# jsansao/voice_synth

Hardware: AMD Instinct MI355X
Metric: synthesised Msamples/s (whole node) at 1/2/4/8 MI355X; RMS vs C ref (higher is better)
Workload: dtype f64

## Files before the change

### voice_synth_amd/csrc/vs_api.c

```c
#include <math.h>
#include <pthread.h>
#include <stdio.h>
#include <stdlib.h>
#include <string.h>
#include <time.h>
#include <unistd.h>

#include "vs_internal.h"

double vs_now_ms(void)
{
  struct timespec ts;
  clock_gettime(CLOCK_MONOTONIC, &ts);
  return 1e3 * (double)ts.tv_sec + 1e-6 * (double)ts.tv_nsec;
}

int vs_ctx_create(int device, vs_ctx **out)
{
  if (!out) return VS_ERR_ARG;
  *out = NULL;
  int count = 0;
  if (hipGetDeviceCount(&count) != hipSuccess || count <= 0) return VS_ERR_NODEVICE;
  if (device < 0 || device >= count) return VS_ERR_NODEVICE;
  hipDeviceProp_t prop;
// ... 366 lines not shown
    b->retired = NULL;
  }
}

int vs_plan_create_impl(vs_ctx *ctx, const vs_lane *lanes, size_t n_lanes, size_t n_samples,
                        int mode, vs_plan **out)
{
  const int filter_only = (mode & VS_PLAN_FILTER_ONLY) ? 1 : 0;
  const int zero_copy = (mode & VS_PLAN_ZERO_COPY) ? 1 : 0;
  if (!ctx || !lanes || !out || n_lanes == 0 || n_samples == 0) return VS_ERR_ARG;
  if (n_lanes > (size_t)0x7FFFFFC0 || n_samples > (size_t)0x7FFFFF00) return VS_ERR_UNSUPPORTED;
  *out = NULL;
  if (!zero_copy) {
    const int wrc = vs_copy_path_warm(ctx);
    if (wrc != VS_OK) return wrc;
  }
  const vs_tuning *tune = &ctx->tuning;
  int rc = VS_OK;
  if (!ctx->planws) {
    ctx->planws = vs_planws_create();
    vs_planws_set_big_allocator(ctx->planws, plan_pinned_alloc, plan_pinned_free, ctx);
  }
  if (!ctx->planws) return VS_ERR_NOMEM;
  VsDevLane *dl = NULL;
  double *costab = NULL;
  size_t costab_len = 0, costab_cap = 0;
  int *row_of_T2 = NULL;
  double *awide = NULL;
  void *small_tmp = NULL;
  VsGroupSlot *gmap = NULL;
  vs_plan *p = NULL;
  const double t_host0 = vs_now_ms();
  VsBatchStats st;
  rc = vs_expand_all_ordered_ws(ctx->planws, lanes, n_lanes, filter_only, &dl, NULL, &st);
  if (rc != VS_OK) goto done;

  int tmax = st.tmax;
  int min_lframe = st.min_lframe;
  const bool any_onoise = st.any_onoise != 0;
  if (!filter_only) {
    row_of_T2 = (int *)malloc(((size_t)st.max_T2 + 1) * sizeof(int));
    if (!row_of_T2) {
      rc = VS_ERR_NOMEM;
      goto done;
    }
    for (int t = 0; t <= st.max_T2; t++) row_of_T2[t] = -1;
    for (size_t l = 0; l < n_lanes; l++) {
      const int T2 = dl[l].T2;
      if (row_of_T2[T2] < 0) {
        if (costab_len + (size_t)T2 > costab_cap) {
          size_t cap = costab_cap ? 2 * costab_cap : 1024;
          while (cap < costab_len + (size_t)T2) cap *= 2;
          double *grown = (double *)realloc(costab, cap * sizeof(double));
          if (!grown) {
            rc = VS_ERR_NOMEM;
            goto done;
          }
          costab = grown;
          costab_cap = cap;
        }
        vs_cos_row(T2, &costab[costab_len]);
        row_of_T2[T2] = (int)costab_len;
        costab_len += (size_t)T2;
      }
      dl[l].tab_off = row_of_T2[T2];
    }
  }
// ... 554 lines not shown
```

### voice_synth_amd/csrc/vs_dev_filter.h

```cpp
#ifndef VS_DEV_FILTER_H
#define VS_DEV_FILTER_H

template <int ARITH>
__device__ __forceinline__ void vs_load_taps(const double *__restrict__ taps, const VsDevLane *__restrict__ L,
                                             double (&a)[VS_ORDER + 1])
{
  const double *__restrict__ row = taps + (size_t)L->tap_row * VS_ORDER;
  a[0] = 1.0;
#pragma unroll
  for (int j = 1; j <= VS_ORDER; ++j) {
    a[j] = (ARITH == VS_ARITH_FMA) ? -row[j - 1] : row[j - 1];
    if (ARITH == VS_ARITH_FMA) asm volatile("" : "+v"(a[j]));
  }
}

__device__ __forceinline__ void vs_unpack8(const vs_u32x4 v, int *x)
{
#pragma unroll
  for (int e = 0; e < 4; ++e) {
    x[2 * e] = (int)(int16_t)(v[e] & 0xFFFFu);
    x[2 * e + 1] = (int)v[e] >> 16;
  }
}

#define VS_ONDW_UNKNOWN 0x7FC00000u
struct VsFramePower {
  float sum;
  float done;
  int tb;
  int len;
  int frame;
  bool bad;
  bool requirk;
  bool force;
  const VsDevLane *lanes;
  float *ondw;
  long ondw_pitch;
  long first_lane;
  int n_lanes;
};
__device__ __forceinline__ double vs_sqrt_rn(double v)
{
  double s = sqrt(v);
  if (!(v > 0.0) || !(s > 0.0)) return s;
  const double r = __builtin_fma(-s, s, v);
  const double up = __longlong_as_double(__double_as_longlong(s) + 1) - s;
  const double dn = s - __longlong_as_double(__double_as_longlong(s) - 1);
  if (r > s * up) s = s + up;
  else if (-r > s * dn) s = s - dn;
  return s;
}
__device__ __forceinline__ float vs_noise_width(float aux, int ni, float snr)
{
  const float sig_power = aux / (float)ni;
  return (float)vs_sqrt_rn((double)(12.0f * sig_power / snr));
}
__device__ __forceinline__ void vs_power_pair(uint32_t w, float &aux)
{
  const float lo = (float)(int)(int16_t)(w & 0xFFFFu), hi = (float)((int)w >> 16);
  aux += lo * lo;
  aux += hi * hi;
}
__device__ __forceinline__ void vs_frame_power_store(const VsFramePower &fp, bool unknown)
{
  const long gl = fp.first_lane + (long)(threadIdx.x & (VS_WAVE - 1));
  if (gl < (long)fp.n_lanes) {
    const VsDevLane *__restrict__ L = fp.lanes + gl;
    const float snr = L->out_snr;
    if (snr > 0.0f)
      fp.ondw[(long)L->row * fp.ondw_pitch + fp.frame] = unknown ? __uint_as_float(VS_ONDW_UNKNOWN) : vs_noise_width(fp.done, fp.len, snr);
  }
}
__device__ __forceinline__ void vs_frame_power_mark(VsFramePower &fp, int t)
{
  const bool ends = fp.tb == t + 1;
  fp.done = ends ? fp.sum : fp.done;
  fp.sum = ends ? 0.0f : fp.sum;
}

template <int ARITH, int KIND, bool PRE1 = false, bool PACKED = false, int WHOLE = -1, bool LATE = false, bool POW = false>
__device__ __forceinline__ void vs_superstep(const double (&a)[VS_ORDER + 1], double (&y)[VS_SS],
                                             double gain, double pre, const int16_t *rp,
                                             const int16_t *__restrict__ irow,
                                             int16_t *__restrict__ orow, int n, int N, bool vec_ok,
                                             int (&outv)[VS_SS], vs_u32x4 (&xnext)[VS_SS / 8],
                                             bool store_ok = true, VsFramePower *fp = nullptr)
{
  static_assert(!POW || (PACKED && WHOLE == 1), "frame powers ride on the eager packing of the branch-free super-step");
  const bool whole = (WHOLE < 0) ? (vec_ok && (n + VS_SS <= N)) : (WHOLE != 0);
  int xin[VS_SS];
  if (KIND == VS_KIND_FILTER) {
    if (whole) {
#pragma unroll
      for (int k = 0; k < VS_SS / 8; ++k) vs_unpack8(xnext[k], &xin[8 * k]);
      if (n + 2 * VS_SS <= N) {
#pragma unroll
        for (int k = 0; k < VS_SS / 8; ++k) xnext[k] = *(const vs_u32x4 *)(irow + n + VS_SS + 8 * k);
      }
    } else {
#pragma unroll
      for (int t = 0; t < VS_SS; ++t) xin[t] = (n + t < N) ? (int)irow[n + t] : 0;
    }
  } else {
#pragma unroll
    for (int t = 0; t < 8; ++t) xin[t] = (int)rp[t * VS_GROUP_LANES];
  }

  constexpr bool EAGER = PACKED && (WHOLE == 1);
  constexpr int PKN = (EAGER && LATE) ? 12 : 4;
  uint32_t pk[PKN];
  auto put8 = [&](int k) {
    if (EAGER && LATE) {
      if (k == VS_SS / 8 - 1) {
#pragma unroll
        for (int c = 0; c < VS_SS / 8; ++c) {
          vs_u32x4 v;
#pragma unroll
          for (int e = 0; e < 4; ++e) v[e] = pk[(4 * c + e) % PKN];
          if (store_ok) *(vs_u32x4 *)(orow + n + 8 * c) = v;
        }
      }
    } else if (EAGER) {
      vs_u32x4 v;
#pragma unroll
      for (int e = 0; e < 4; ++e) v[e] = pk[e];
      if (store_ok) *(vs_u32x4 *)(orow + n + 8 * k) = v;
    } else if (whole) {
      vs_u32x4 v;
#pragma unroll
      for (int e = 0; e < 4; ++e)
        v[e] = PACKED ? vs_clamp_pack16(outv[8 * k + 2 * e], outv[8 * k + 2 * e + 1])
                      : vs_pack16(outv[8 * k + 2 * e], outv[8 * k + 2 * e + 1]);
      if (store_ok) *(vs_u32x4 *)(orow + n + 8 * k) = v;
    } else {
#pragma unroll
      for (int t = 8 * k; t < 8 * k + 8; ++t) {
        int v = outv[t];
        if (PACKED) v = (v > 32767) ? 32767 : ((v < -32767) ? -32767 : v);
        if (store_ok && (n + t < N)) orow[n + t] = (int16_t)v;
      }
    }
  };

  if (KIND == VS_KIND_SOURCE) {
#pragma unroll
    for (int t = 8; t < VS_SS; ++t) xin[t] = (int)rp[t * VS_GROUP_LANES];
#pragma unroll
    for (int t = 0; t < VS_SS; ++t) outv[t] = xin[t];
#pragma unroll
    for (int k = 0; k < VS_SS / 8; ++k) put8(k);
  } else {
    const double ym1 = y[VS_SS - 1];
    int qhi = 0x7FFFFFFF;
    uint32_t qlo = 0u;
#pragma unroll
    for (int t = 0; t < VS_SS; ++t) {
      if (KIND != VS_KIND_FILTER && (t & 7) == 0) {
        if (t + 8 < VS_SS) {
#pragma unroll
          for (int u = t + 8; u < t + 16; ++u) xin[u] = (int)rp[u * VS_GROUP_LANES];
        }
        asm volatile(".p2align 3" ::"v"(xin[t]), "v"(xin[t + 1]), "v"(xin[t + 2]), "v"(xin[t + 3]), "v"(xin[t + 4]),
                     "v"(xin[t + 5]), "v"(xin[t + 6]), "v"(xin[t + 7]));
      }
      double acc;
      const double y1 = y[(t + VS_SS - 1) % VS_SS];
      if (ARITH == VS_ARITH_EXACT) {
        acc = __builtin_fma((double)xin[t], gain, -(a[1] * y1));
#pragma unroll
        for (int j = 2; j <= VS_ORDER; ++j) acc = acc - a[j] * y[(t + VS_SS - j) % VS_SS];
      } else {
        acc = (double)xin[t] * gain;
        double p0 = acc, p1 = a[2] * y[(t + VS_SS - 2) % VS_SS];
#pragma unroll
        for (int j = 3; j <= VS_ORDER; ++j) {
          const double yj = y[(t + VS_SS - j) % VS_SS];
          if (j & 1) p0 = __builtin_fma(a[j], yj, p0);
          else p1 = __builtin_fma(a[j], yj, p1);
        }
        acc = __builtin_fma(a[1], y1, p0 + p1);
      }
      const double o = PRE1 ? (acc - y1)
                            : ((ARITH == VS_ARITH_EXACT) ? (acc - pre * y1) : __builtin_fma(-pre, y1, acc));
      if (ARITH == VS_ARITH_FMA && PACKED) {
        outv[t] = (int)__builtin_rint(o);
        asm volatile("" : "+v"(outv[t]));
      } else {
        outv[t] = PACKED ? vs_round2int_half_down_unclamped(o) : vs_round2int_half_down(o);
        asm volatile("" : "+v"(outv[t]));
        const int ohi = __double2hiint(o);
        const uint32_t olo = (uint32_t)__double2loint(o);
        qhi = (ohi < qhi) ? ohi : qhi;
        qlo = (olo > qlo) ? olo : qlo;
// ... 117 lines not shown
```

### voice_synth_amd/csrc/vs_kernels.hip

```cpp
#include <hip/hip_runtime.h>
#include <stdint.h>

#include "../../include/voice_synth.h"
#include "vs_device.h"

#include "vs_dev_primitives.h"
#include "vs_dev_generator.h"
#include "vs_dev_filter.h"


__device__ __forceinline__ void vs_load_cfg(const VsDevLane *__restrict__ L, VsCfg &c, VsGen &s)
{
  c.jitter = L->jitter; c.shimmer = L->shimmer; c.K = L->K; c.Kvar = L->Kvar;
  c.DC = L->DC; c.noise = L->noise; c.t_hi = L->t_hi; c.t_lo = L->t_lo;
  c.a_hi = L->a_hi; c.a_lo = L->a_lo;
  c.amp = L->amp; c.P = L->P; c.T2 = L->T2; c.tab_off = 0;
  c.dcs = L->dcs;
  c.thr = L->thr;
  c.flags = L->flags; c.key0 = L->key0; c.key1 = L->key1;
  s.d = 0u;
  s.dp0 = 0.0f; s.ds0 = 0.0f;
  s.T4 = 0; s.T = c.P; s.g = 0; s.wpos = 0; s.cyc = 0;
  s.amp_next = 0.0f; s.S_next = 0.0f; s.K_next = 0.0f; s.pend = false; s.posted = 0;
}
// ... 109 lines not shown
    VS_DIAG_ADD(dg, 6)
  }
#ifdef VS_DIAG
  if (args.diag && lane == 0) {
#pragma unroll
    for (int k = 0; k < 8; ++k) args.diag[(size_t)blockIdx.x * 8 + k] = dg.acc[k];
  }
#endif

  if (KIND != VS_KIND_FILTER && args.ncyc && valid) args.ncyc[row] = s.cyc;
}

#if VS_GROUP_LANES == VS_WAVE
#ifdef VS_POLL_SLEEP
#define VS_POLL_SLEEP_2 VS_POLL_SLEEP
#define VS_POLL_SLEEP_3 VS_POLL_SLEEP
#else
#define VS_POLL_SLEEP_2 32
#define VS_POLL_SLEEP_3 8
#endif
template <bool THREE>
__device__ __forceinline__ void vs_poll_sleep()
{
  if (THREE) __builtin_amdgcn_s_sleep(VS_POLL_SLEEP_3);
  else __builtin_amdgcn_s_sleep(VS_POLL_SLEEP_2);
}

struct VsGroup {
  const VsDevLane *L;
  int16_t *ring;
  double *ltab;
  int *gpub, *npub;
  VsOrderBox ord;
  long group, row;
  int lane, N, C;
  int ltab_entries;
  bool valid;
};

template <bool SPLIT>
__device__ __forceinline__ void vs_generator_wave(const VsKernelArgs &args, const VsGroup &g)
{
  const int lane = g.lane, N = g.N, C = g.C;
  VsCfg c;
  VsGen s;
  VsDiag dg;
#ifdef VS_DIAG
#pragma unroll
  for (int k = 0; k < 8; ++k) dg.acc[k] = 0;
  dg.rounds = dg.attend = 0;
  dg.t = vs_stamp();
#endif
  vs_load_cfg(g.L, c, s);
  vs_stage_cos_rows(g.L, c, g.ltab, args.costab, g.ltab_entries, lane, g.valid, args);
  __builtin_amdgcn_fence(__ATOMIC_RELEASE, "workgroup");
  VsRoundKeys rk;
  if (!SPLIT) vs_round_keys(c.key0, c.key1, rk);
  int spins = 0;
  int prev_seen = -1, prev_taken = -1;
  bool dirty = true;
  const bool withhold = args.fault == VS_FAULT_WITHHOLD_PROGRESS;
  while (!withhold) {
#ifdef VS_TIMING_GENERATOR_ONLY
    const int n_seen = s.g;
#else
    const int n_seen = __hip_atomic_load(&g.npub[lane], __ATOMIC_RELAXED, __HIP_MEMORY_SCOPE_WORKGROUP);
#endif
// ... 85 lines not shown
        taken += 1;
        VS_LDS_RELEASE();
        __hip_atomic_store(&g.ord.otak[lane], taken, __ATOMIC_RELAXED, __HIP_MEMORY_SCOPE_WORKGROUP);
        const int T3 = w1 & 0xFFFF, T = (int)((unsigned)w1 >> 16);
        const int m = T - T3;
        __hip_atomic_store(&g.gpub[lane], gend + T3, __ATOMIC_RELAXED, __HIP_MEMORY_SCOPE_WORKGROUP);
        if (__any(m > 0)) {
          vs_noise_trips<true, true>(g.ring, C, lane, rk, vs_noise_consts(NDW, dcs), d0, m, wpos, T3, gend,
                                     &g.gpub[lane]);
        }
        gend += T;
        wpos += T;
        if (wpos >= C) wpos -= C;
      }
      spins = 0;
      VS_DIAG_ADD(dg, 4)
    } else {
      vs_poll_sleep<true>();
      VS_DIAG_ADD(dg, 6)
      if (++spins > args.spin_limit) {
        if (args.err && lane == 0) atomicOr(args.err, 4);
        break;
      }
    }
  }
#ifdef VS_DIAG
  if (args.diag && lane == 0) {
    args.diag[(size_t)g.group * 16 + 11] = dg.acc[4];
    args.diag[(size_t)g.group * 16 + 12] = dg.acc[6];
  }
#endif
}

template <int ARITH, bool PRE1, bool PARTIAL, bool POW>
__device__ __forceinline__ void vs_filter_wave(const VsKernelArgs &args, const VsGroup &g)
{
  const int lane = g.lane, N = g.N, C = g.C;
  const VsDevLane *__restrict__ L = g.L;
  int16_t *ring = g.ring;
  int *gpub = g.gpub, *npub = g.npub;
  const bool valid = g.valid;
  if (args.ws_filter_prio >= 3) __builtin_amdgcn_s_setprio(3);
  else if (args.ws_filter_prio == 2) __builtin_amdgcn_s_setprio(2);
  else if (args.ws_filter_prio == 1) __builtin_amdgcn_s_setprio(1);
  constexpr bool F32 = (ARITH == VS_ARITH_F32);
  constexpr int DARITH = F32 ? VS_ARITH_FMA : ARITH;
  VsF32Filter f32;
  double a[VS_ORDER + 1];
  if (F32) vs_f32_load(args.taps, L, f32);
  else vs_load_taps<DARITH>(args.taps, L, a);
  const double gain = L->gain;
  const double pre = L->pre;
  int16_t *orow = args.out + g.row * args.out_pitch;
  const int ready_min = (args.ready_min > 0) ? args.ready_min : __builtin_amdgcn_readfirstlane(L->ready_min);
#ifdef VS_DIAG
  VsDiag dg;
#pragma unroll
  for (int k = 0; k < 8; ++k) dg.acc[k] = 0;
  dg.t = vs_stamp();
#endif
  if (!PARTIAL || ready_min >= VS_WAVE) {
    double y[VS_SS];
#pragma unroll
    for (int j = 0; j < VS_SS; ++j) y[j] = 0.0;
    bool gave_up = false;
    int rslot = 0;
    auto await = [&](int n) {
      for (int polls = 0; !gave_up; ++polls) {
#ifdef VS_TIMING_FILTER_ONLY
        const int g_seen = N;
#else
        const int g_seen = __hip_atomic_load(&gpub[lane], __ATOMIC_RELAXED, __HIP_MEMORY_SCOPE_WORKGROUP);
#endif
        const bool ready = !valid || (g_seen - n >= VS_SS) || (g_seen >= N);
        if (__all(ready)) break;
        vs_poll_sleep<!PARTIAL>();
        VS_DIAG_ADD(dg, 6)
        if (polls > args.spin_limit) {
          if (args.err && lane == 0) atomicOr(args.err, 2);
          gave_up = true;
        }
      }
      __builtin_amdgcn_fence(__ATOMIC_ACQUIRE, "workgroup");
    };
    auto release = [&](int n_done) {
      rslot += VS_SS;
      if (rslot >= C) rslot = 0;
      VS_LDS_RELEASE();
      __hip_atomic_store(&npub[lane], n_done, __ATOMIC_RELAXED, __HIP_MEMORY_SCOPE_WORKGROUP);
    };
    if (!valid) orow = args.sink;
    const int n_whole = (args.vec_ok != 0) ? (N / VS_SS) * VS_SS : 0;
    VsFramePower fp;
    int f_len = 0, f_left = 0;
    if (POW) {
      fp.sum = fp.done = 0.0f;
      fp.frame = 0;
      fp.bad = fp.requirk = false;
      fp.lanes = args.lanes;
      fp.ondw = args.ondw;
      fp.ondw_pitch = args.ondw_pitch;
      fp.first_lane = g.group * VS_WAVE;
      fp.n_lanes = args.n_lanes;
      f_len = f_left = (args.pow_lframe < N) ? args.pow_lframe : N;
    }
    int n = 0;
    for (; n < n_whole; n += VS_SS) {
      VS_DIAG_ADD(dg, 7)
      await(n);
      int outv[VS_SS];
      vs_u32x4 xpre[VS_SS / 8];
      if (POW) {
        fp.tb = (f_left <= VS_SS) ? f_left : 0;
        fp.len = f_len;
        fp.force = (args.fault == VS_FAULT_REROUND) && ((n / VS_SS) % 7 == 3);
      }
      if constexpr (F32)
        vs_superstep_f32<PRE1, 1, POW>(f32, ring + rslot * VS_WAVE + lane, orow, n, N, true, &fp);
      else
        vs_superstep<DARITH, VS_KIND_SYNTH, PRE1, true, 1, PARTIAL, POW>(a, y, gain, pre, ring + rslot * VS_WAVE + lane, nullptr, orow, n,
                                                                         N, true, outv, xpre, true, &fp);
      if (POW) {
        if (fp.tb) {
          vs_frame_power_store(fp, fp.bad || fp.requirk);
          fp.frame += 1;
          fp.bad = fp.requirk;
          const int rest = N - (n + fp.tb);
          f_len = (args.pow_lframe < rest) ? args.pow_lframe : rest;
          f_left = f_len - (VS_SS - fp.tb);
        } else {
          fp.bad = fp.bad || fp.requirk;
          f_left -= VS_SS;
        }
        fp.requirk = false;
      }
      release(n + VS_SS);
      VS_DIAG_ADD(dg, 0)
    }
    if (POW && valid) args.odone[g.row] = fp.frame;
    for (; n < N; n += VS_SS) {
      VS_DIAG_ADD(dg, 7)
      await(n);
      int outv[VS_SS];
      vs_u32x4 xpre[VS_SS / 8];
      if constexpr (F32)
        vs_superstep_f32<PRE1, 0, false>(f32, ring + rslot * VS_WAVE + lane, orow, n, N, true);
      else
        vs_superstep<DARITH, VS_KIND_SYNTH, PRE1, true, 0>(a, y, gain, pre, ring + rslot * VS_WAVE + lane, nullptr, orow, n,
                                                           N, false, outv, xpre, true);
      release(n + VS_SS);
      VS_DIAG_ADD(dg, 0)
    }
  } else {
    if (POW && valid) args.odone[g.row] = 0;
    double y[VS_SS];
#pragma unroll
    for (int j = 0; j < VS_SS; ++j) y[j] = 0.0;
    int n = 0, rslot = 0, spins = 0;
    bool live = valid;
    while (__any(live)) {
      VS_DIAG_ADD(dg, 7)
#ifdef VS_TIMING_FILTER_ONLY
      const int g_seen = N;
#else
      const int g_seen = __hip_atomic_load(&gpub[lane], __ATOMIC_RELAXED, __HIP_MEMORY_SCOPE_WORKGROUP);
#endif
      __builtin_amdgcn_fence(__ATOMIC_ACQUIRE, "workgroup");
      const bool ready = live && ((g_seen - n >= VS_SS) || (g_seen >= N));
      const int n_live = __builtin_popcountll(__ballot(live));
      const int n_ready = __builtin_popcountll(__ballot(ready));
      if ((n_ready > 0) && (n_ready * 64 >= n_live * ready_min)) {
        const bool inside = (args.vec_ok != 0) && (n + VS_SS <= N);
        if (__all(!ready || inside)) {
          if (ready) {
            int outv[VS_SS];
            vs_u32x4 xpre[VS_SS / 8];
            if constexpr (F32)
              vs_superstep_f32<PRE1, 1, false>(f32, ring + rslot * VS_WAVE + lane, orow, n, N, true);
            else
              vs_superstep<DARITH, VS_KIND_SYNTH, PRE1, true, 1, PARTIAL>(a, y, gain, pre, ring + rslot * VS_WAVE + lane, nullptr, orow,
                                                                          n, N, true, outv, xpre);
          }
        } else {
          if (ready) {
            int outv[VS_SS];
            vs_u32x4 xpre[VS_SS / 8];
            if constexpr (F32)
              vs_superstep_f32<PRE1, 0, false>(f32, ring + rslot * VS_WAVE + lane, orow, n, N, true);
            else
              vs_superstep<DARITH, VS_KIND_SYNTH, PRE1, true>(a, y, gain, pre, ring + rslot * VS_WAVE + lane, nullptr, orow,
                                                              n, N, args.vec_ok != 0, outv, xpre);
          }
        }
        if (ready) {
          rslot += VS_SS;
          if (rslot >= C) rslot = 0;
          n += VS_SS;
          if (n >= N) live = false;
        }
        VS_LDS_RELEASE();
        __hip_atomic_store(&npub[lane], n, __ATOMIC_RELAXED, __HIP_MEMORY_SCOPE_WORKGROUP);
        spins = 0;
        VS_DIAG_ADD(dg, 0)
      } else {
        vs_poll_sleep<!PARTIAL>();
        VS_DIAG_ADD(dg, 6)
        if (++spins > args.spin_limit) {
          if (args.err && lane == 0) atomicOr(args.err, 2);
          break;
        }
      }
    }
  }
#ifdef VS_DIAG
  if (args.diag && lane == 0) {
    args.diag[(size_t)g.group * 16 + 8] = dg.acc[0];
    args.diag[(size_t)g.group * 16 + 14] = dg.acc[6];
    args.diag[(size_t)g.group * 16 + 15] = dg.acc[7];
  }
#endif
}

template <int ARITH, bool PRE1, int ROLES, bool POW>
__device__ __forceinline__ void vs_synth_ws_body(const VsKernelArgs &args)
{
  extern __shared__ __attribute__((aligned(16))) int16_t lds_base[];

  const int widx = (int)threadIdx.x >> 6;
  int ngroups, role, slot;
  if (ROLES == 3 && args.ws_layout == VS_WS_LAYOUT_SPREAD_2X3) {
    const int simd = widx & 3, second = widx >> 2;
    ngroups = 2;
    slot = simd >> 1;
    role = (simd & 1) ? (second ? 1 : 0) : (second ? -1 : 2);
  } else {
    ngroups = (int)blockDim.x / (ROLES * VS_WAVE);
    role = widx / ngroups;
    slot = widx - role * ngroups;
  }
  VsGroup g;
  g.lane = (int)threadIdx.x & (VS_WAVE - 1);
  g.group = (long)blockIdx.x * (long)ngroups + slot;
  g.C = args.ring_slots;
  g.ltab_entries = args.ltab_entries;
  g.ring = lds_base + (size_t)slot * (size_t)(args.ws_pair_bytes / sizeof(int16_t));
  if (args.group_map) {
    const VsGroupSlot gs = args.group_map[(size_t)blockIdx.x * (size_t)ngroups + (size_t)slot];
    g.group = (gs.group >= 0) ? (long)gs.group : (((long)args.n_lanes + VS_WAVE - 1) / VS_WAVE);
    g.C = __builtin_amdgcn_readfirstlane(gs.ring_slots);
    g.ring = lds_base + (size_t)__builtin_amdgcn_readfirstlane(gs.lds_off) / sizeof(int16_t);
    g.ltab_entries = __builtin_amdgcn_readfirstlane(gs.ltab_entries);
  }
  const long gl = g.group * VS_WAVE + g.lane;
  g.valid = gl < (long)args.n_lanes;
  g.L = args.lanes + (g.valid ? gl : (long)args.n_lanes - 1);
  g.N = args.n_samples;
  g.ltab = (double *)(g.ring + (size_t)(g.C + VS_TRASH_ROWS) * VS_WAVE);
  g.gpub = (int *)(g.ltab + g.ltab_entries);
  g.npub = g.gpub + VS_WAVE;
  g.ord.oseq = g.npub + VS_WAVE;
  g.ord.otak = g.ord.oseq + VS_WAVE;
  g.ord.w = g.ord.otak + VS_WAVE;
  g.row = (long)g.L->row;

  if (role == 0) {
    g.gpub[g.lane] = 0;
    g.npub[g.lane] = 0;
    if (ROLES == 3) {
      g.ord.oseq[g.lane] = 0;
      g.ord.otak[g.lane] = 0;
    }
  }
  __syncthreads();
  if (role < 0) return;
  if (g.group * VS_WAVE >= (long)args.n_lanes) return;

#ifdef VS_TIMING_GENERATOR_ONLY
  if (role == ROLES - 1) return;
#endif
#ifdef VS_TIMING_FILTER_ONLY
  if (role != ROLES - 1) return;
#endif
  if (role == ROLES - 1) vs_filter_wave<ARITH, PRE1, ROLES == 2, POW>(args, g);
  else if (ROLES == 3 && role == 1) vs_noise_wave(args, g);
  else vs_generator_wave<ROLES == 3>(args, g);
}
template <int ARITH, bool PRE1, int ROLES>
__global__ void __launch_bounds__(ROLES * 4 * VS_WAVE) vs_synth_ws_kernel(VsKernelArgs args)
{
  vs_synth_ws_body<ARITH, PRE1, ROLES, false>(args);
}
template <int ARITH, bool PRE1, int ROLES>
__global__ void __launch_bounds__(ROLES * 4 * VS_WAVE) vs_synth_ws_pow_kernel(VsKernelArgs args)
{
  vs_synth_ws_body<ARITH, PRE1, ROLES, true>(args);
}

__device__ __forceinline__ void vs_power8(const vs_u32x4 v, float &aux)
{
#pragma unroll
  for (int e = 0; e < 4; ++e) {
    const float lo = (float)(int)(int16_t)(v[e] & 0xFFFFu), hi = (float)((int)v[e] >> 16);
    aux += lo * lo;
    aux += hi * hi;
  }
}

template <bool VEC>
__device__ __forceinline__ float vs_frame_width(const VsKernelArgs &args, const VsDevLane *__restrict__ L, long row, int fr, float snr)
{
  const int N = args.n_samples;
  const int Lframe = L->Lframe;
  const long f0 = (long)fr * Lframe;
  if (f0 >= N) return __uint_as_float(VS_ONDW_UNKNOWN);
  const int left = N - (int)f0;
  const int ni = (left < Lframe) ? left : Lframe;
// ... 565 lines not shown
```

### voice_synth_amd/csrc/vs_planhost.c

```c
#include <math.h>
#include <pthread.h>
#include <signal.h>
#include <stdlib.h>
#include <string.h>
#include <unistd.h>

#include "vs_planhost.h"

uint32_t vs_lframe_magic(int Lframe)
{
  if (Lframe < 2) return 0u;
  int k = 0;
  while (((uint64_t)1 << k) < (uint64_t)Lframe) k++;
  return (uint32_t)((((uint64_t)1 << (31 + k)) / (uint64_t)Lframe) + 1u);
}

int vs_lane_taps(const vs_lane *lane, double *A)
{
  for (int j = 0; j < VS_MAX_NCOEF; j++) A[j] = 0.0;
  if (lane->vowel != VS_VOWEL_CUSTOM) return vs_vowel_coefficients(lane->vowel, A);
  int order = 0;
  const int rc = vs_lane_order(lane, &order);
  if (rc != VS_OK) return rc;
  for (int j = 0; j <= order; j++) A[j] = lane->A[j];
// ... 114 lines not shown
  } else if (vs_vowel_index(lane->vowel) < 0) {
    return (lane->vowel == 'A' || lane->vowel == 'I' || lane->vowel == 'U') ? VS_ERR_UNSUPPORTED : VS_ERR_RANGE;
  }
  if (lane->fs <= 0) return VS_ERR_RANGE;
  memset(d, 0, sizeof(*d));
  d->tap_row = (lane->vowel == VS_VOWEL_CUSTOM) ? -1 : vs_vowel_index(lane->vowel);
  d->gain = (double)lane->gain;
  d->pre = (double)lane->pre_emphasis;
  d->row = row;
  d->out_snr = lane->out_snr;
  {
    const unsigned long nSamplesPerSec = (unsigned long)lane->fs;
    const int milisec1 = (int)(nSamplesPerSec * 0.001 / 2.0) * 2;
    d->Lframe = 50 * milisec1;
    d->lframe_magic = vs_lframe_magic(d->Lframe);
  }
  if (lane->out_snr > 0 && d->Lframe <= 0) return VS_ERR_UNSUPPORTED;
  d->okey0 = (uint32_t)lane->out_seed;
  d->okey1 = (uint32_t)(lane->out_seed >> 32);
  return VS_OK;
}

#define VS_EXPAND_THREADS 16
typedef struct ExpandJob {
  const vs_lane *lanes;
  VsDevLane *dl;
  const uint32_t *order;
  size_t lo, hi;
  int filter_only;
  int rc;
  size_t bad;
  VsBatchStats st;
  uint64_t *key;
  uint64_t key_or, key_and;
} ExpandJob;

static void stats_init(VsBatchStats *st)
{
  memset(st, 0, sizeof(*st));
  st->tmax = 1;
  st->pre1 = 1;
}
static void stats_lane(VsBatchStats *st, const vs_lane *lane, const VsDevLane *d)
{
  if (d->T2 > st->max_T2) st->max_T2 = d->T2;
  if (d->tbound > st->tmax) st->tmax = d->tbound;
  if (d->Lframe > 0 && (st->min_lframe == 0 || d->Lframe < st->min_lframe)) st->min_lframe = d->Lframe;
  if (d->Lframe > st->max_lframe) st->max_lframe = d->Lframe;
  if (d->Lframe <= 0) st->no_lframe = 1;
  if (d->out_snr > 0) st->any_onoise = 1;
  if (d->pre != 1.0) st->pre1 = 0;
  if (vs_lane_is_wide(lane)) st->wide = 1;
  if (d->tap_row < 0) st->n_custom++;
  if (d->flags & VS_DF_NOISE) st->n_noisy++;
}
static void stats_merge(VsBatchStats *a, const VsBatchStats *b)
{
  if (b->max_T2 > a->max_T2) a->max_T2 = b->max_T2;
  if (b->tmax > a->tmax) a->tmax = b->tmax;
  if (b->min_lframe > 0 && (a->min_lframe == 0 || b->min_lframe < a->min_lframe)) a->min_lframe = b->min_lframe;
  if (b->max_lframe > a->max_lframe) a->max_lframe = b->max_lframe;
  a->no_lframe |= b->no_lframe;
  a->any_onoise |= b->any_onoise;
  a->pre1 &= b->pre1;
  a->wide |= b->wide;
  a->n_noisy += b->n_noisy;
// ... 200 lines not shown
    rec_release(ws);
    ws->rec_big = (ws->big_alloc != NULL) && n >= VS_TEAM_MIN_LANES;
    ws->rec[0] = rec_alloc(ws, 0, n);
    if (!ws->rec[0]) return VS_ERR_NOMEM;
    ws->rec_lanes = n;
  }
  if (need_order) {
    if (!ws->rec[1]) {
      ws->rec[1] = rec_alloc(ws, 1, ws->rec_lanes);
      if (!ws->rec[1]) return VS_ERR_NOMEM;
    }
    if (ws->idx_lanes < n) {
      free(ws->idx[0]);
      free(ws->idx[1]);
      ws->idx_lanes = 0;
      ws->idx[0] = (uint32_t *)malloc(n * sizeof(uint32_t));
      ws->idx[1] = (uint32_t *)malloc(n * sizeof(uint32_t));
      if (!ws->idx[0] || !ws->idx[1]) return VS_ERR_NOMEM;
      ws->idx_lanes = n;
    }
    if (!ws->count) ws->count = (size_t *)malloc(65537 * sizeof(size_t));
    if (!ws->count) return VS_ERR_NOMEM;
  }
  if (ws->key_lanes < n) {
    free(ws->key);
    ws->key_lanes = 0;
    ws->key = (uint64_t *)malloc(n * sizeof(uint64_t));
    if (!ws->key) return VS_ERR_NOMEM;
    ws->key_lanes = n;
  }
  return VS_OK;
}

static uint64_t record_order_key(const VsDevLane *d)
{
  return ((uint64_t)(uint32_t)d->P << 36) | ((uint64_t)(uint32_t)d->T2 << 8) |
         (uint64_t)(d->flags & (VS_DF_JITTER | VS_DF_SHIMMER | VS_DF_NOISE));
}

static void expand_range(void *arg)
{
  ExpandJob *j = (ExpandJob *)arg;
  j->rc = VS_OK;
  j->bad = (size_t)-1;
  j->key_or = 0;
  j->key_and = ~(uint64_t)0;
  stats_init(&j->st);
  for (size_t i = j->lo; i < j->hi; i++) {
    const size_t l = j->order ? (size_t)j->order[i] : i;
    const int rc = j->filter_only ? vs_expand_filter_lane(&j->lanes[l], (int32_t)l, &j->dl[i])
                                  : vs_expand_lane(&j->lanes[l], (int32_t)l, &j->dl[i]);
    if (rc != VS_OK) {
      if (l < j->bad) {
        j->rc = rc;
        j->bad = l;
      }
      if (!j->order) break;
      continue;
    }
    stats_lane(&j->st, &j->lanes[l], &j->dl[i]);
    if (j->key) {
      const uint64_t k = record_order_key(&j->dl[i]);
      j->key[i] = k;
      j->key_or |= k;
      j->key_and &= k;
    }
  }
}

typedef struct GatherJob {
  const VsDevLane *in;
  VsDevLane *out;
  const uint32_t *order;
  size_t lo, hi;
} GatherJob;
static void gather_range(void *arg)
{
  GatherJob *j = (GatherJob *)arg;
  for (size_t i = j->lo; i < j->hi; i++) j->out[i] = j->in[j->order[i]];
}

static int jobs_for(size_t n_lanes, int parallel)
{
  if (!parallel) return 1;
  size_t n = (n_lanes + VS_JOB_LANES - 1) / VS_JOB_LANES;
  if (n > VS_MAX_JOBS) n = VS_MAX_JOBS;
  return n ? (int)n : 1;
}

static int expand_pass(VsTeam *team, const vs_lane *lanes, VsDevLane *dl, size_t n_lanes, int filter_only,
                       const uint32_t *order, uint64_t *key, uint64_t *varying, VsBatchStats *stats)
{
  ExpandJob jobs[VS_MAX_JOBS];
  const int n_jobs = jobs_for(n_lanes, team != NULL);
  const size_t per = (n_lanes + (size_t)n_jobs - 1) / (size_t)n_jobs;
  int made = 0;
  for (int t = 0; t < n_jobs; t++) {
    const size_t lo = (size_t)t * per, hi = (lo + per < n_lanes) ? lo + per : n_lanes;
    if (lo >= hi) break;
    ExpandJob *j = &jobs[made++];
    j->lanes = lanes;
    j->dl = dl;
    j->order = order;
    j->key = key;
    j->lo = lo;
    j->hi = hi;
    j->filter_only = filter_only;
  }
  team_run(team, expand_range, jobs, sizeof(ExpandJob), made);
  int rc = VS_OK;
  size_t bad = (size_t)-1;
  uint64_t k_or = 0, k_and = ~(uint64_t)0;
  VsBatchStats all;
  stats_init(&all);
  for (int t = 0; t < made; t++) {
    if (jobs[t].rc != VS_OK && jobs[t].bad < bad) {
      rc = jobs[t].rc;
      bad = jobs[t].bad;
    }
    stats_merge(&all, &jobs[t].st);
    k_or |= jobs[t].key_or;
    k_and &= jobs[t].key_and;
  }
  if (stats) *stats = all;
  if (varying) *varying = made ? (k_or ^ k_and) : 0;
  return rc;
}

static uint32_t *radix_order(const uint64_t *key, uint64_t varying, size_t n_lanes, uint32_t *a, uint32_t *b, size_t *count)
{
  for (size_t l = 0; l < n_lanes; l++) a[l] = (uint32_t)l;
  for (int shift = 0; shift < 64; shift += 16) {
    if (!((varying >> shift) & 0xFFFFu)) continue;
    memset(count, 0, 65537 * sizeof(size_t));
    for (size_t i = 0; i < n_lanes; i++) count[((key[a[i]] >> shift) & 0xFFFFu) + 1]++;
    for (size_t d = 0; d < 65536; d++) count[d + 1] += count[d];
    for (size_t i = 0; i < n_lanes; i++) b[count[(key[a[i]] >> shift) & 0xFFFFu]++] = a[i];
    uint32_t *sw = a;
    a = b;
    b = sw;
  }
  return a;
}

int vs_expand_all_ordered_ws(VsPlanWs *ws, const vs_lane *lanes, size_t n_lanes, int filter_only, VsDevLane **dl_out,
                             int *reordered, VsBatchStats *stats)
{
  if (!ws || !lanes || !dl_out || n_lanes == 0) return VS_ERR_ARG;
  if (reordered) *reordered = 0;
  const int may_order = !filter_only && n_lanes >= 2 && n_lanes <= 0xFFFFFFFFu;
  int rc = ws_reserve(ws, n_lanes, 0);
  if (rc != VS_OK) return rc;
  if (n_lanes >= VS_TEAM_MIN_LANES && !ws->team) ws->team = team_create();
  VsTeam *team = (n_lanes >= VS_TEAM_MIN_LANES) ? ws->team : NULL;
  uint64_t varying = 0;
  rc = expand_pass(team, lanes, ws->rec[0], n_lanes, filter_only, NULL, may_order ? ws->key : NULL, &varying, stats);
  if (rc != VS_OK) return rc;
  *dl_out = ws->rec[0];
  if (!may_order || !varying) return VS_OK;
  rc = ws_reserve(ws, n_lanes, 1);
  if (rc != VS_OK) return rc;
  const uint32_t *order = radix_order(ws->key, varying, n_lanes, ws->idx[0], ws->idx[1], ws->count);
  GatherJob jobs[VS_MAX_JOBS];
  const int n_jobs = jobs_for(n_lanes, team != NULL);
  const size_t per = (n_lanes + (size_t)n_jobs - 1) / (size_t)n_jobs;
  int made = 0;
  for (int t = 0; t < n_jobs; t++) {
    const size_t lo = (size_t)t * per, hi = (lo + per < n_lanes) ? lo + per : n_lanes;
    if (lo >= hi) break;
    GatherJob *j = &jobs[made++];
    j->in = ws->rec[0];
    j->out = ws->rec[1];
    j->order = order;
    j->lo = lo;
    j->hi = hi;
  }
  team_run(team, gather_range, jobs, sizeof(GatherJob), made);
  *dl_out = ws->rec[1];
  if (reordered) *reordered = 1;
  return VS_OK;
}

static int expand_into(const vs_lane *lanes, VsDevLane *dl, size_t n_lanes, int filter_only, int ordered, int *reordered,
                       VsBatchStats *stats)
{
  if (!lanes || !dl) return VS_ERR_ARG;
  if (reordered) *reordered = 0;
  if (n_lanes == 0) {
    if (stats) stats_init(stats);
    return VS_OK;
  }
  if (!ordered) {
    VsTeam *team = (n_lanes >= VS_TEAM_MIN_LANES) ? team_create() : NULL;
    const int rc = expand_pass(team, lanes, dl, n_lanes, filter_only, NULL, NULL, NULL, stats);
    team_destroy(team);
    return rc;
  }
  VsPlanWs *ws = vs_planws_create();
  if (!ws) return VS_ERR_NOMEM;
  VsDevLane *out = NULL;
  const int rc = vs_expand_all_ordered_ws(ws, lanes, n_lanes, filter_only, &out, reordered, stats);
  if (rc == VS_OK) memcpy(dl, out, n_lanes * sizeof(VsDevLane));
  vs_planws_destroy(ws);
  return rc;
}

int vs_expand_all(const vs_lane *lanes, VsDevLane *dl, size_t n_lanes, int filter_only)
{
  return expand_into(lanes, dl, n_lanes, filter_only, 0, NULL, NULL);
}

int vs_expand_all_stats(const vs_lane *lanes, VsDevLane *dl, size_t n_lanes, int filter_only, VsBatchStats *stats)
{
  return expand_into(lanes, dl, n_lanes, filter_only, 0, NULL, stats);
}

static uint64_t lane_order_key(const vs_lane *lane)
{
  uint64_t P = 0, T2 = 0;
  if (lane->fs > 0 && lane->F0 > 0.0f) {
    const float q = (float)lane->fs / lane->F0;
    if (q >= 0.0f && q < 67108864.0f) P = (uint64_t)(int)q;
  }
  if (lane->cq >= 0.0f && lane->cq <= 1.0f) {
    const double t2 = ceil(0.5 * lane->cq * (double)P);
    if (t2 >= 0.0 && t2 < 67108864.0) T2 = (uint64_t)t2;
  }
// ... 163 lines not shown
```

### voice_synth_amd/csrc/vs_planhost.h

```cpp
#ifndef VS_PLANHOST_H
#define VS_PLANHOST_H

#include <stdbool.h>
#include <stddef.h>
#include <stdint.h>

#include "../../include/voice_synth.h"
#include "vs_device.h"

#ifdef __cplusplus
extern "C" {
#endif
int vs_lane_taps(const vs_lane *lane, double *A);
int vs_vowel_index(int vowel);
int vs_vowel_by_index(int index);
int vs_tap_table_build(const vs_lane *lanes, VsDevLane *dl, size_t n_lanes, size_t n_custom, double **taps, size_t *rows);
bool vs_lane_is_wide(const vs_lane *lane);
uint32_t vs_lframe_magic(int Lframe);
int vs_expand_lane(const vs_lane *lane, int32_t row, VsDevLane *d);
int vs_expand_filter_lane(const vs_lane *lane, int32_t row, VsDevLane *d);
typedef struct VsBatchStats {
  int max_T2;
  int tmax;
  int min_lframe;
  int max_lframe;
  int no_lframe;
  int any_onoise;
  int pre1;
  int wide;
  size_t n_noisy;
  size_t n_custom;
} VsBatchStats;
int vs_expand_all(const vs_lane *lanes, VsDevLane *dl, size_t n_lanes, int filter_only);
int vs_expand_all_stats(const vs_lane *lanes, VsDevLane *dl, size_t n_lanes, int filter_only, VsBatchStats *stats);
int vs_kernel_order(const vs_lane *lanes, size_t n_lanes, uint32_t **order);
int vs_expand_all_ordered(const vs_lane *lanes, VsDevLane *dl, size_t n_lanes, int *reordered, VsBatchStats *stats);
typedef struct VsPlanWs VsPlanWs;
VsPlanWs *vs_planws_create(void);
void vs_planws_destroy(VsPlanWs *ws);
typedef void *(*vs_planws_alloc_fn)(void *user, size_t bytes);
typedef void (*vs_planws_free_fn)(void *user, void *ptr);
void vs_planws_set_big_allocator(VsPlanWs *ws, vs_planws_alloc_fn alloc, vs_planws_free_fn release, void *user);
int vs_expand_all_ordered_ws(VsPlanWs *ws, const vs_lane *lanes, size_t n_lanes, int filter_only, VsDevLane **dl,
                             int *reordered, VsBatchStats *stats);
void vs_cos_row(int T2, double *row);
int vs_ring_policy_for(int group_lanes, int tmax, int cap, int *slots, int *ready_min, int request, double depth);
int vs_ring_policy(int tmax, int cap, int *slots, int *ready_min);
int vs_ring_slots_for(int tmax, int *slots);
int vs_mixed_rings_build(const VsDevLane *dl, size_t n_lanes, int floor_slots, VsGroupSlot **gmap, size_t *n_wg,
                         size_t *max_lds, int *c_min, int *c_max);
#ifdef __cplusplus
}
#endif
#endif
```

Before: 403,300.

## Sort lanes by tap row and keep uniform filter taps in scalar registers

The host ordering key now also includes the tap row, so waves are more likely to share one filter. When every valid lane in a wave has the same taps, the filter wave reads them once with readlane and keeps them in scalar registers. This frees vector registers in the double-precision recurrence. Kernel-argument fields used by the frame-power path are reloaded from the kernarg segment instead of being kept live, with optional compile-time store and prefetch variants. The cost is an extra template instantiation and a wave-level branch. Sorting by taps may also break the existing pitch/period grouping.

```diff
diff --git a/voice_synth_amd/csrc/vs_api.c b/voice_synth_amd/csrc/vs_api.c
--- a/voice_synth_amd/csrc/vs_api.c
+++ b/voice_synth_amd/csrc/vs_api.c
@@ -422,7 +422,7 @@
   vs_plan *p = NULL;
   const double t_host0 = vs_now_ms();
   VsBatchStats st;
-  rc = vs_expand_all_ordered_ws(ctx->planws, lanes, n_lanes, filter_only, &dl, NULL, &st);
+  rc = vs_expand_all_grouped_ws(ctx->planws, lanes, n_lanes, filter_only, 1, &dl, NULL, &st);
   if (rc != VS_OK) goto done;
 
   int tmax = st.tmax;
diff --git a/voice_synth_amd/csrc/vs_dev_filter.h b/voice_synth_amd/csrc/vs_dev_filter.h
--- a/voice_synth_amd/csrc/vs_dev_filter.h
+++ b/voice_synth_amd/csrc/vs_dev_filter.h
@@ -1,12 +1,27 @@
 #ifndef VS_DEV_FILTER_H
 #define VS_DEV_FILTER_H
 
-template <int ARITH>
+template <int ARITH, bool UNIFORM = false>
 __device__ __forceinline__ void vs_load_taps(const double *__restrict__ taps, const VsDevLane *__restrict__ L,
                                              double (&a)[VS_ORDER + 1])
 {
+  a[0] = 1.0;
+  if (UNIFORM) {
+    const double *__restrict__ row = taps + (size_t)__builtin_amdgcn_readfirstlane(L->tap_row) * VS_ORDER;
+    const int ln = (int)threadIdx.x & (VS_WAVE - 1);
+    const double mine = row[(ln < VS_ORDER) ? ln : 0];
+    const int mlo = __double2loint(mine), mhi = __double2hiint(mine);
+#pragma unroll
+    for (int j = 1; j <= VS_ORDER; ++j) {
+      const int lo = __builtin_amdgcn_readlane(mlo, j - 1);
+      int hi = __builtin_amdgcn_readlane(mhi, j - 1);
+      if (ARITH == VS_ARITH_FMA) hi ^= (int)0x80000000u;
+      a[j] = __hiloint2double(hi, lo);
+      asm volatile("" : "+s"(a[j]));
+    }
+    return;
+  }
   const double *__restrict__ row = taps + (size_t)L->tap_row * VS_ORDER;
-  a[0] = 1.0;
 #pragma unroll
   for (int j = 1; j <= VS_ORDER; ++j) {
     a[j] = (ARITH == VS_ARITH_FMA) ? -row[j - 1] : row[j - 1];
@@ -33,11 +48,7 @@
   bool bad;
   bool requirk;
   bool force;
-  const VsDevLane *lanes;
-  float *ondw;
-  long ondw_pitch;
   long first_lane;
-  int n_lanes;
 };
 __device__ __forceinline__ double vs_sqrt_rn(double v)
 {
@@ -63,12 +74,15 @@
 }
 __device__ __forceinline__ void vs_frame_power_store(const VsFramePower &fp, bool unknown)
 {
+  const volatile VsKernelArgs *ka = (const volatile VsKernelArgs *)__builtin_amdgcn_kernarg_segment_ptr();
   const long gl = fp.first_lane + (long)(threadIdx.x & (VS_WAVE - 1));
-  if (gl < (long)fp.n_lanes) {
-    const VsDevLane *__restrict__ L = fp.lanes + gl;
+  if (gl < (long)ka->n_lanes) {
+    const VsDevLane *__restrict__ L = (const VsDevLane *)ka->lanes + gl;
     const float snr = L->out_snr;
-    if (snr > 0.0f)
-      fp.ondw[(long)L->row * fp.ondw_pitch + fp.frame] = unknown ? __uint_as_float(VS_ONDW_UNKNOWN) : vs_noise_width(fp.done, fp.len, snr);
+    if (snr > 0.0f) {
+      float *ondw = (float *)ka->ondw;
+      ondw[(long)L->row * (long)ka->ondw_pitch + fp.frame] = unknown ? __uint_as_float(VS_ONDW_UNKNOWN) : vs_noise_width(fp.done, fp.len, snr);
+    }
   }
 }
 __device__ __forceinline__ void vs_frame_power_mark(VsFramePower &fp, int t)
@@ -78,7 +92,8 @@
   fp.sum = ends ? 0.0f : fp.sum;
 }
 
-template <int ARITH, int KIND, bool PRE1 = false, bool PACKED = false, int WHOLE = -1, bool LATE = false, bool POW = false>
+template <int ARITH, int KIND, bool PRE1 = false, bool PACKED = false, int WHOLE = -1, bool LATE = false, bool POW = false,
+          int PKSETS = 1, bool UPFRONT = false>
 __device__ __forceinline__ void vs_superstep(const double (&a)[VS_ORDER + 1], double (&y)[VS_SS],
                                              double gain, double pre, const int16_t *rp,
                                              const int16_t *__restrict__ irow,
@@ -103,11 +118,11 @@
     }
   } else {
 #pragma unroll
-    for (int t = 0; t < 8; ++t) xin[t] = (int)rp[t * VS_GROUP_LANES];
+    for (int t = 0; t < (UPFRONT ? VS_SS : 8); ++t) xin[t] = (int)rp[t * VS_GROUP_LANES];
   }
 
   constexpr bool EAGER = PACKED && (WHOLE == 1);
-  constexpr int PKN = (EAGER && LATE) ? 12 : 4;
+  constexpr int PKN = (EAGER && LATE) ? 12 : ((EAGER && PKSETS == 2) ? 8 : 4);
   uint32_t pk[PKN];
   auto put8 = [&](int k) {
     if (EAGER && LATE) {
@@ -123,7 +138,7 @@
     } else if (EAGER) {
       vs_u32x4 v;
 #pragma unroll
-      for (int e = 0; e < 4; ++e) v[e] = pk[e];
+      for (int e = 0; e < 4; ++e) v[e] = pk[(4 * k + e) % PKN];
       if (store_ok) *(vs_u32x4 *)(orow + n + 8 * k) = v;
     } else if (whole) {
       vs_u32x4 v;
@@ -156,9 +171,13 @@
 #pragma unroll
     for (int t = 0; t < VS_SS; ++t) {
       if (KIND != VS_KIND_FILTER && (t & 7) == 0) {
-        if (t + 8 < VS_SS) {
+        if (!UPFRONT && t + 8 < VS_SS) {
 #pragma unroll
           for (int u = t + 8; u < t + 16; ++u) xin[u] = (int)rp[u * VS_GROUP_LANES];
+        }
+        if (UPFRONT && t == 0) {
+#pragma unroll
+          for (int u = 8; u < VS_SS; ++u) asm volatile("" ::"v"(xin[u]));
         }
         asm volatile(".p2align 3" ::"v"(xin[t]), "v"(xin[t + 1]), "v"(xin[t + 2]), "v"(xin[t + 3]), "v"(xin[t + 4]),
                      "v"(xin[t + 5]), "v"(xin[t + 6]), "v"(xin[t + 7]));
diff --git a/voice_synth_amd/csrc/vs_kernels.hip b/voice_synth_amd/csrc/vs_kernels.hip
--- a/voice_synth_amd/csrc/vs_kernels.hip
+++ b/voice_synth_amd/csrc/vs_kernels.hip
@@ -165,7 +165,8 @@
   double *ltab;
   int *gpub, *npub;
   VsOrderBox ord;
-  long group, row;
+  long group;
+  int row;
   int lane, N, C;
   int ltab_entries;
   bool valid;
@@ -317,9 +318,20 @@
 #endif
 }
 
-template <int ARITH, bool PRE1, bool PARTIAL, bool POW>
+__device__ __forceinline__ const volatile VsKernelArgs *vs_args_again()
+{
+  return (const volatile VsKernelArgs *)__builtin_amdgcn_kernarg_segment_ptr();
+}
+#ifndef VS_UNI_STORES
+#define VS_UNI_STORES 0
+#endif
+template <int ARITH, bool PRE1, bool PARTIAL, bool POW, bool UNI>
 __device__ __forceinline__ void vs_filter_wave(const VsKernelArgs &args, const VsGroup &g)
 {
+  constexpr bool U3 = UNI && !PARTIAL;
+  constexpr bool LATE = PARTIAL || (U3 && (VS_UNI_STORES & 3) == 1);
+  constexpr int PKSETS = (U3 && (VS_UNI_STORES & 3) == 2) ? 2 : 1;
+  constexpr bool UPFRONT = U3 && (VS_UNI_STORES & 4) != 0;
   const int lane = g.lane, N = g.N, C = g.C;
   const VsDevLane *__restrict__ L = g.L;
   int16_t *ring = g.ring;
@@ -333,10 +345,11 @@
   VsF32Filter f32;
   double a[VS_ORDER + 1];
   if (F32) vs_f32_load(args.taps, L, f32);
-  else vs_load_taps<DARITH>(args.taps, L, a);
-  const double gain = L->gain;
-  const double pre = L->pre;
-  int16_t *orow = args.out + g.row * args.out_pitch;
+  else vs_load_taps<DARITH, UNI>(args.taps, L, a);
+  double gain = L->gain;
+  double pre = L->pre;
+  if (UNI) asm volatile("" : "+v"(gain), "+v"(pre));
+  int16_t *orow = args.out + (long)g.row * args.out_pitch;
   const int ready_min = (args.ready_min > 0) ? args.ready_min : __builtin_amdgcn_readfirstlane(L->ready_min);
 #ifdef VS_DIAG
   VsDiag dg;
@@ -362,7 +375,8 @@
         vs_poll_sleep<!PARTIAL>();
         VS_DIAG_ADD(dg, 6)
         if (polls > args.spin_limit) {
-          if (args.err && lane == 0) atomicOr(args.err, 2);
+          int *err = (int *)vs_args_again()->err;
+          if (err && lane == 0) atomicOr(err, 2);
           gave_up = true;
         }
       }
@@ -382,11 +396,7 @@
       fp.sum = fp.done = 0.0f;
       fp.frame = 0;
       fp.bad = fp.requirk = false;
-      fp.lanes = args.lanes;
-      fp.ondw = args.ondw;
-      fp.ondw_pitch = args.ondw_pitch;
       fp.first_lane = g.group * VS_WAVE;
-      fp.n_lanes = args.n_lanes;
       f_len = f_left = (args.pow_lframe < N) ? args.pow_lframe : N;
     }
     int n = 0;
@@ -403,8 +413,8 @@
       if constexpr (F32)
         vs_superstep_f32<PRE1, 1, POW>(f32, ring + rslot * VS_WAVE + lane, orow, n, N, true, &fp);
       else
-        vs_superstep<DARITH, VS_KIND_SYNTH, PRE1, true, 1, PARTIAL, POW>(a, y, gain, pre, ring + rslot * VS_WAVE + lane, nullptr, orow, n,
-                                                                         N, true, outv, xpre, true, &fp);
+        vs_superstep<DARITH, VS_KIND_SYNTH, PRE1, true, 1, LATE, POW, PKSETS, UPFRONT>(a, y, gain, pre, ring + rslot * VS_WAVE + lane,
+                                                                                       nullptr, orow, n, N, true, outv, xpre, true, &fp);
       if (POW) {
         if (fp.tb) {
           vs_frame_power_store(fp, fp.bad || fp.requirk);
@@ -422,7 +432,11 @@
       release(n + VS_SS);
       VS_DIAG_ADD(dg, 0)
     }
-    if (POW && valid) args.odone[g.row] = fp.frame;
+    if (POW && valid) ((int32_t *)vs_args_again()->odone)[(long)g.row] = fp.frame;
+    if (UNI && !F32) {
+#pragma unroll
+      for (int j = 1; j <= VS_ORDER; ++j) asm volatile("" : "+v"(a[j]));
+    }
     for (; n < N; n += VS_SS) {
       VS_DIAG_ADD(dg, 7)
       await(n);
@@ -437,7 +451,7 @@
       VS_DIAG_ADD(dg, 0)
     }
   } else {
-    if (POW && valid) args.odone[g.row] = 0;
+    if (POW && valid) ((int32_t *)vs_args_again()->odone)[(long)g.row] = 0;
     double y[VS_SS];
 #pragma unroll
     for (int j = 0; j < VS_SS; ++j) y[j] = 0.0;
@@ -491,7 +505,8 @@
         vs_poll_sleep<!PARTIAL>();
         VS_DIAG_ADD(dg, 6)
         if (++spins > args.spin_limit) {
-          if (args.err && lane == 0) atomicOr(args.err, 2);
+          int *err = (int *)vs_args_again()->err;
+          if (err && lane == 0) atomicOr(err, 2);
           break;
         }
       }
@@ -506,12 +521,30 @@
 #endif
 }
 
+template <int ARITH, bool PRE1, bool PARTIAL, bool POW>
+__device__ __forceinline__ void vs_filter_role(const VsKernelArgs &args, const VsGroup &g)
+{
+  if constexpr (ARITH == VS_ARITH_F32) {
+    vs_filter_wave<ARITH, PRE1, PARTIAL, POW, false>(args, g);
+  } else {
+    const int tr = g.L->tap_row;
+    const bool same = !g.valid || (tr == __builtin_amdgcn_readfirstlane(tr));
+    constexpr bool MIXED_POW = POW && (PARTIAL || ARITH != VS_ARITH_EXACT);
+    if (__all(same)) {
+      vs_filter_wave<ARITH, PRE1, PARTIAL, POW, true>(args, g);
+    } else {
+      if (POW && !MIXED_POW && g.valid) ((int32_t *)vs_args_again()->odone)[g.row] = 0;
+      vs_filter_wave<ARITH, PRE1, PARTIAL, MIXED_POW, false>(args, g);
+    }
+  }
+}
+
 template <int ARITH, bool PRE1, int ROLES, bool POW>
 __device__ __forceinline__ void vs_synth_ws_body(const VsKernelArgs &args)
 {
   extern __shared__ __attribute__((aligned(16))) int16_t lds_base[];
 
-  const int widx = (int)threadIdx.x >> 6;
+  const int widx = __builtin_amdgcn_readfirstlane((int)threadIdx.x >> 6);
   int ngroups, role, slot;
   if (ROLES == 3 && args.ws_layout == VS_WS_LAYOUT_SPREAD_2X3) {
     const int simd = widx & 3, second = widx >> 2;
@@ -546,7 +579,7 @@
   g.ord.oseq = g.npub + VS_WAVE;
   g.ord.otak = g.ord.oseq + VS_WAVE;
   g.ord.w = g.ord.otak + VS_WAVE;
-  g.row = (long)g.L->row;
+  g.row = g.L->row;
 
   if (role == 0) {
     g.gpub[g.lane] = 0;
@@ -566,7 +599,7 @@
 #ifdef VS_TIMING_FILTER_ONLY
   if (role != ROLES - 1) return;
 #endif
-  if (role == ROLES - 1) vs_filter_wave<ARITH, PRE1, ROLES == 2, POW>(args, g);
+  if (role == ROLES - 1) vs_filter_role<ARITH, PRE1, ROLES == 2, POW>(args, g);
   else if (ROLES == 3 && role == 1) vs_noise_wave(args, g);
   else vs_generator_wave<ROLES == 3>(args, g);
 }
diff --git a/voice_synth_amd/csrc/vs_planhost.c b/voice_synth_amd/csrc/vs_planhost.c
--- a/voice_synth_amd/csrc/vs_planhost.c
+++ b/voice_synth_amd/csrc/vs_planhost.c
@@ -170,6 +170,7 @@
   size_t bad;
   VsBatchStats st;
   uint64_t *key;
+  int by_taps;
   uint64_t key_or, key_and;
 } ExpandJob;
 
@@ -436,10 +437,18 @@
   return VS_OK;
 }
 
+#define VS_KEY_OPT_SHIFT 5
 static uint64_t record_order_key(const VsDevLane *d)
 {
   return ((uint64_t)(uint32_t)d->P << 36) | ((uint64_t)(uint32_t)d->T2 << 8) |
-         (uint64_t)(d->flags & (VS_DF_JITTER | VS_DF_SHIMMER | VS_DF_NOISE));
+         ((uint64_t)(d->flags & (VS_DF_JITTER | VS_DF_SHIMMER | VS_DF_NOISE)) << VS_KEY_OPT_SHIFT);
+}
+#define VS_KEY_TAP_SHIFT 0
+#define VS_KEY_TAP_CUSTOM 31u
+static uint64_t record_tap_key(const VsDevLane *d)
+{
+  const uint32_t t = (d->tap_row >= 0 && (uint32_t)d->tap_row < VS_KEY_TAP_CUSTOM) ? (uint32_t)d->tap_row : VS_KEY_TAP_CUSTOM;
+  return (uint64_t)t << VS_KEY_TAP_SHIFT;
 }
 
 static void expand_range(void *arg)
@@ -464,7 +473,7 @@
     }
     stats_lane(&j->st, &j->lanes[l], &j->dl[i]);
     if (j->key) {
-      const uint64_t k = record_order_key(&j->dl[i]);
+      const uint64_t k = record_order_key(&j->dl[i]) | (j->by_taps ? record_tap_key(&j->dl[i]) : 0);
       j->key[i] = k;
       j->key_or |= k;
       j->key_and &= k;
@@ -493,7 +502,7 @@
 }
 
 static int expand_pass(VsTeam *team, const vs_lane *lanes, VsDevLane *dl, size_t n_lanes, int filter_only,
-                       const uint32_t *order, uint64_t *key, uint64_t *varying, VsBatchStats *stats)
+                       const uint32_t *order, uint64_t *key, int by_taps, uint64_t *varying, VsBatchStats *stats)
 {
   ExpandJob jobs[VS_MAX_JOBS];
   const int n_jobs = jobs_for(n_lanes, team != NULL);
@@ -507,6 +516,7 @@
     j->dl = dl;
     j->order = order;
     j->key = key;
+    j->by_taps = by_taps;
     j->lo = lo;
     j->hi = hi;
     j->filter_only = filter_only;
@@ -550,6 +560,12 @@
 int vs_expand_all_ordered_ws(VsPlanWs *ws, const vs_lane *lanes, size_t n_lanes, int filter_only, VsDevLane **dl_out,
                              int *reordered, VsBatchStats *stats)
 {
+  return vs_expand_all_grouped_ws(ws, lanes, n_lanes, filter_only, 0, dl_out, reordered, stats);
+}
+
+int vs_expand_all_grouped_ws(VsPlanWs *ws, const vs_lane *lanes, size_t n_lanes, int filter_only, int by_taps,
+                             VsDevLane **dl_out, int *reordered, VsBatchStats *stats)
+{
   if (!ws || !lanes || !dl_out || n_lanes == 0) return VS_ERR_ARG;
   if (reordered) *reordered = 0;
   const int may_order = !filter_only && n_lanes >= 2 && n_lanes <= 0xFFFFFFFFu;
@@ -558,7 +574,7 @@
   if (n_lanes >= VS_TEAM_MIN_LANES && !ws->team) ws->team = team_create();
   VsTeam *team = (n_lanes >= VS_TEAM_MIN_LANES) ? ws->team : NULL;
   uint64_t varying = 0;
-  rc = expand_pass(team, lanes, ws->rec[0], n_lanes, filter_only, NULL, may_order ? ws->key : NULL, &varying, stats);
+  rc = expand_pass(team, lanes, ws->rec[0], n_lanes, filter_only, NULL, may_order ? ws->key : NULL, by_taps, &varying, stats);
   if (rc != VS_OK) return rc;
   *dl_out = ws->rec[0];
   if (!may_order || !varying) return VS_OK;
@@ -596,7 +612,7 @@
   }
   if (!ordered) {
     VsTeam *team = (n_lanes >= VS_TEAM_MIN_LANES) ? team_create() : NULL;
-    const int rc = expand_pass(team, lanes, dl, n_lanes, filter_only, NULL, NULL, NULL, stats);
+    const int rc = expand_pass(team, lanes, dl, n_lanes, filter_only, NULL, NULL, 0, NULL, stats);
     team_destroy(team);
     return rc;
   }
diff --git a/voice_synth_amd/csrc/vs_planhost.h b/voice_synth_amd/csrc/vs_planhost.h
--- a/voice_synth_amd/csrc/vs_planhost.h
+++ b/voice_synth_amd/csrc/vs_planhost.h
@@ -43,6 +43,8 @@
 void vs_planws_set_big_allocator(VsPlanWs *ws, vs_planws_alloc_fn alloc, vs_planws_free_fn release, void *user);
 int vs_expand_all_ordered_ws(VsPlanWs *ws, const vs_lane *lanes, size_t n_lanes, int filter_only, VsDevLane **dl,
                              int *reordered, VsBatchStats *stats);
+int vs_expand_all_grouped_ws(VsPlanWs *ws, const vs_lane *lanes, size_t n_lanes, int filter_only, int by_taps,
+                             VsDevLane **dl, int *reordered, VsBatchStats *stats);
 void vs_cos_row(int T2, double *row);
 int vs_ring_policy_for(int group_lanes, int tmax, int cap, int *slots, int *ready_min, int request, double depth);
 int vs_ring_policy(int tmax, int cap, int *slots, int *ready_min);
```

New measurement: 420,100, median of 6. +4.2%, better.
